# zouyuoz/SVS-UNet-PyTorch

Hardware: AMD Instinct MI355X
Metric: spectrogram-tiles/sec (512x128) U-Net fwd+bwd (L1 train step incl. Adam) (higher is better)
Workload: dtype f32; 1 GPU; train.py L1-loss step, 512x128 tiles, batch 64 per GPU; global_batch=64, parallelism=dp1, mode=train

## Files before the change

### svs_unet_pytorch_amd/csrc/gemm_conv.hip

```cpp
#include <stdlib.h>
#include <string.h>

#include <mutex>
#include <type_traits>
#include <vector>
#include "conv_geom.h"
#include "gemm_pipeline.h"
#include "mfma_split.h"

enum { MODE_GATHER = SVS_MODE_GATHER, MODE_PARITY = SVS_MODE_PARITY };

struct ConvGemmArgs {
  const float* x; long ldx;
  int B, H, W, C;
  const float* wp;
  const float* bias;
  const float* scale;
  const float* shift;
  float slope;
  float* y; long ldy;
  int Ho, Wo, N;
  int accumulate;
  int ksplit;
  float* slab;
// ... 4 lines not shown

struct ConvBal {
  int enabled;
  int npos[4];
  unsigned first[4][65];
  unsigned char nsplit[4][64];
  unsigned char* rowsplit;
};
struct ConvNoBal {};

__device__ __forceinline__ void conv_put(const ConvGemmArgs& p, float v, float* dst, const float* bias, const float* scale, const float* shift,
                                         int n, float& ssum, float& ssq) {
  if (p.bias) v += bias[n];
  if (p.scale) {
    v = v * scale[n] + shift[n];
    v = v > 0.f ? v : v * p.slope;
  }
  if (p.accumulate) v += *dst;
  *dst = v;
  ssum += v;
  ssq += v * v;
}

template <int MODE, int BM, int BN, int WM, int WN, bool UNI, bool SKIP, bool SPLIT, int PF>
__global__ __launch_bounds__(256) void conv_gemm_kernel(ConvGemmArgs p, std::conditional_t<SKIP, ConvBal, ConvNoBal> bal) {
  static_assert(SKIP || !UNI, "the position-uniform form is a form of the tap-skipping kernel");
  constexpr int TM = BM / WM / 16;
  constexpr int TN = BN / WN / 16;
  constexpr int RA = (BM + 63) / 64;
  constexpr int RB = (BN + 63) / 64;
  static_assert(WM * WN == 4, "4 waves");
  static_assert(TM >= 1 && TN >= 1, "tile");

  __shared__ __attribute__((aligned(16))) float As[2][BM * 16];
  __shared__ __attribute__((aligned(16))) float Bs[2][BN * 16];

  const int t = threadIdx.x;
  const int lane = t & 63, wave = t >> 6;
  const int wm = wave / WN, wn = wave % WN;
  const int lrow = lane & 15, q = lane >> 4;

  int bx = blockIdx.x, by = blockIdx.y, bz = blockIdx.z;
  int nsplit = p.ksplit;
  bool balanced = false;
  int upos = -1, ub0 = 0;
  if constexpr (SKIP) {
    if (bal.enabled) {
      balanced = true;
      const unsigned bid = blockIdx.x;
      int c = 0;
      if (MODE == MODE_PARITY) c = (bid >= bal.first[1][0]) + (bid >= bal.first[2][0]) + (bid >= bal.first[3][0]);
      const unsigned f = lane < bal.npos[c] ? bal.first[c][lane] : 0xFFFFFFFFu;
      const int pos = __builtin_amdgcn_readfirstlane(__builtin_popcountll(__ballot(f <= bid)) - 1);
      nsplit = bal.nsplit[c][pos];
      const int ntn = p.N / BN, per = nsplit * ntn;
      const int within = (int)(bid - bal.first[c][pos]);
      const int i = within / per, rem = within - i * per;
      by = rem / ntn;
      bx = (pos * (p.B / BM) + i) * ntn + (rem - by * ntn);
      bz = c;
      upos = pos; ub0 = i * BM;
    }
  }
  const SvsConvClass cls = svs_conv_class<MODE>(bz, p.Ho, p.Wo);
  const int ph = cls.ph, pw = cls.pw, nth = cls.nth, ntw = cls.ntw;
  const int Ha = cls.Ha, Wa = cls.Wa;
  const float* const wp = p.wp + (long)cls.tap0 * p.N * p.C;
  const int ntaps = nth * ntw;
  const long M = (long)p.B * Ha * Wa;
  const int ntile_n = p.N / BN;
  const long m0 = (long)(bx / ntile_n) * BM;
  const int n0 = (bx % ntile_n) * BN;
  if (m0 >= M) {
    if (p.stats && p.ksplit == 1) {
      float* out = p.stats + ((long)bz * (gridDim.x / ntile_n) + bx / ntile_n) * 2 * p.N + n0;
      for (int c = threadIdx.x; c < BN; c += 256) { out[c] = 0.f; out[p.N + c] = 0.f; }
    }
    return;
  }
  const int cpt = p.C >> 4;
  const int nkt = ntaps * cpt;
  int kt_begin = (int)((long)nkt * by / nsplit);
  int kt_end = (int)((long)nkt * (by + 1) / nsplit);
  const long Kw = (long)ntaps * p.C;

  const int chunk = t & 3;
  constexpr unsigned OOB = 0x80000000u;
  unsigned a_voff[RA], a_mask[RA];
  unsigned umask = 0x1FFFFFFu;
  int uhq = 0, uwq = 0;
  if constexpr (UNI) {
    if (upos < 0) {
      upos = (int)((unsigned)m0 / (unsigned)p.B);
      ub0 = (int)((unsigned)m0 - (unsigned)upos * (unsigned)p.B);
    }
    uwq = (int)((unsigned)upos / (unsigned)Ha);
    uhq = upos - uwq * Ha;
    const int h0 = svs_conv_anchor<MODE>(uhq), w0 = svs_conv_anchor<MODE>(uwq);
    umask = svs_tap_mask<MODE>(h0, w0, nth, ntw, p.H, p.W);
    const unsigned base = (unsigned)((((long)h0 * p.W + w0) * p.ldx + chunk * 4) * 4);
    const unsigned per_image = (unsigned)(((long)p.H * p.W * p.ldx) * 4);
#pragma unroll
    for (int r = 0; r < RA; ++r) {
      const int row = (t >> 2) + 64 * r;
      a_voff[r] = (BM % 64 == 0 || row < BM) ? base + (unsigned)(ub0 + row) * per_image : OOB;
      a_mask[r] = 0;
    }
  } else {
#pragma unroll
  for (int r = 0; r < RA; ++r) {
    const int row = (t >> 2) + 64 * r;
    const long m = m0 + row;
    const bool ok = (row < BM) && (m < M);
    const SvsConvRow g = svs_conv_row<SKIP>(ok ? (unsigned)m : 0u, p.B, Ha, Wa);
    const int h0 = svs_conv_anchor<MODE>(g.hq), w0 = svs_conv_anchor<MODE>(g.wq);
    a_voff[r] = ok ? (unsigned)(((((long)g.b * p.H + h0) * p.W + w0) * p.ldx + chunk * 4) * 4) : OOB;
    a_mask[r] = ok ? svs_tap_mask<MODE>(h0, w0, nth, ntw, p.H, p.W) : 0u;
  }
  }
  if (SKIP) {
    if constexpr (!UNI) {
      __shared__ unsigned umask_s;
      if (t == 0) umask_s = 0;
      __syncthreads();
      unsigned mine = 0;
#pragma unroll
      for (int r = 0; r < RA; ++r) mine |= a_mask[r];
      if (mine) atomicOr(&umask_s, mine);
      __syncthreads();
      umask = __builtin_amdgcn_readfirstlane(umask_s);
    }
    if (balanced) {
      const int nvk = __builtin_popcount(umask) << p.cpt_shift;
      const int vb = (int)((long)nvk * by / nsplit), ve = (int)((long)nvk * (by + 1) / nsplit);
      auto kt_of = [&](int v) -> int {
        unsigned m = umask;
        for (int r = v >> p.cpt_shift; r > 0; --r) m &= m - 1;
        return (__builtin_ctz(m) << p.cpt_shift) | (v & (cpt - 1));
      };
      kt_begin = vb < nvk ? kt_of(vb) : nkt;
      kt_end = ve < nvk ? kt_of(ve) : nkt;
    }
  }
  unsigned b_voff[RB];
#pragma unroll
  for (int r = 0; r < RB; ++r) {
    const int row = (t >> 2) + 64 * r;
    b_voff[r] = (row < BN) ? (unsigned)(((long)(n0 + row) * Kw + chunk * 4) * 4) : OOB;
  }
  const __amdgpu_buffer_rsrc_t rx = __builtin_amdgcn_make_buffer_rsrc((void*)(p.x - svs_tap_base_shift<MODE>(p.W, p.ldx)), 0, OOB, 0x00020000);
  const __amdgpu_buffer_rsrc_t rw = __builtin_amdgcn_make_buffer_rsrc((void*)wp, 0, OOB, 0x00020000);

  f32x4 ra[PF][RA], rb[PF][RB];
  auto load_tile = [&](int kt, auto setc) __attribute__((always_inline)) {
    constexpr int set_ = decltype(setc)::value;
    int tap, cc;
    if (SKIP || !p.tap_inner) {
      if (p.cpt_shift >= 0) { tap = kt >> p.cpt_shift; cc = kt & (cpt - 1); }
      else { tap = kt / cpt; cc = kt - tap * cpt; }
    } else {
      cc = (ntaps == 25) ? kt / 25 : (ntaps == 9) ? kt / 9 : (ntaps == 6) ? kt / 6 : kt >> 2;
      tap = kt - cc * ntaps;
    }
    const int th = svs_tap_row(tap, ntw);
    const int tw = tap - th * ntw;
    const int pix = svs_tap_pix<MODE>(th, tw, p.W);
    const int soff_a = __builtin_amdgcn_readfirstlane((int)((pix * p.ldx + (cc << 4)) * 4));
    const int soff_b = __builtin_amdgcn_readfirstlane((int)(((long)tap * p.C + (cc << 4)) * 4));
#pragma unroll
    for (int r = 0; r < RA; ++r) {
      const unsigned vo = (UNI || ((a_mask[r] >> tap) & 1u)) ? a_voff[r] : OOB;
      ra[set_][r] = __builtin_bit_cast(f32x4, __builtin_amdgcn_raw_buffer_load_b128(rx, (int)vo, soff_a, 0));
    }
#pragma unroll
    for (int r = 0; r < RB; ++r)
      rb[set_][r] = __builtin_bit_cast(f32x4, __builtin_amdgcn_raw_buffer_load_b128(rw, (int)b_voff[r], soff_b, 0));
  };
  auto store_tile = [&](int buf, auto setc) __attribute__((always_inline)) {
#pragma unroll
    for (int r = 0; r < RA; ++r) {
      const int row = (t >> 2) + 64 * r;
      if (BM % 64 == 0 || row < BM) *(f32x4*)(&As[buf][row * 16 + swz(row, chunk) * 4]) = ra[decltype(setc)::value][r];
    }
#pragma unroll
    for (int r = 0; r < RB; ++r) {
      const int row = (t >> 2) + 64 * r;
      if (BN % 64 == 0 || row < BN) *(f32x4*)(&Bs[buf][row * 16 + swz(row, chunk) * 4]) = rb[decltype(setc)::value][r];
    }
  };
  f32x4 acc[TM][TN];
#pragma unroll
  for (int i = 0; i < TM; ++i)
#pragma unroll
    for (int j = 0; j < TN; ++j) acc[i][j] = (f32x4){0.f, 0.f, 0.f, 0.f};

  auto first_valid = [&](int k) -> int {
    if (!SKIP || k >= kt_end) return k;
    const int tp = k >> p.cpt_shift;
    if ((umask >> tp) & 1u) return k;
    const unsigned rest = umask >> (tp + 1);
    if (!rest) return kt_end;
    const int nk = (tp + 1 + __builtin_ctz(rest)) << p.cpt_shift;
    return nk < kt_end ? nk : kt_end;
  };
  auto multiply = [&](int buf) __attribute__((always_inline)) {
    f32x4 fa[TM], fb[TN];
#pragma unroll
    for (int i = 0; i < TM; ++i) {
      const int row = wm * (TM * 16) + i * 16 + lrow;
      fa[i] = *(const f32x4*)(&As[buf][row * 16 + swz(row, q) * 4]);
    }
#pragma unroll
    for (int j = 0; j < TN; ++j) {
      const int row = wn * (TN * 16) + j * 16 + lrow;
      fb[j] = *(const f32x4*)(&Bs[buf][row * 16 + swz(row, q) * 4]);
    }
    if constexpr (SPLIT) {
      SvsSplitA sa[TM];
      SvsSplitB sb[TN];
#pragma unroll
      for (int i = 0; i < TM; ++i) sa[i] = svs_split_a(fa[i][0], fa[i][1], fa[i][2], fa[i][3]);
#pragma unroll
      for (int j = 0; j < TN; ++j) sb[j] = svs_split_b(fb[j][0], fb[j][1], fb[j][2], fb[j][3]);
      svs_mma_split<TM, TN>(acc, sa, sb);
    } else {
#pragma unroll
      for (int k = 0; k < 4; ++k)
#pragma unroll
        for (int i = 0; i < TM; ++i)
#pragma unroll
          for (int j = 0; j < TN; ++j)
            acc[i][j] = __builtin_amdgcn_mfma_f32_16x16x4f32(fa[i][k], fb[j][k], acc[i][j], 0, 0, 0);
    }
  };
  svs_k_loop<PF>(first_valid(kt_begin), kt_end, [&](int k) { return first_valid(k + 1); }, load_tile, store_tile, multiply);

  const bool split = p.ksplit > 1;
  float ssum[TN], ssq[TN];
#pragma unroll
  for (int j = 0; j < TN; ++j) { ssum[j] = 0.f; ssq[j] = 0.f; }
  float* const slab = split ? p.slab + (long)by * ((long)p.B * p.Ho * p.Wo) * p.N : nullptr;
  bool mark_rows = false;
  if constexpr (SKIP) mark_rows = balanced && by == 0 && n0 == 0 && wn == 0;
  if constexpr (UNI) {
    const long HoWo = (long)p.Ho * p.Wo;
    const long pix0 = svs_out_pixel<MODE>(0, uhq, uwq, ph, pw, p.Ho, p.Wo) + (long)(ub0 + wm * (TM * 16) + q * 4) * HoWo;
    const int ncol = n0 + wn * (TN * 16) + lrow;
    const long rstride = HoWo * (split ? (long)p.N : p.ldy);
    float* const out = split ? slab + pix0 * p.N + ncol : p.y + pix0 * p.ldy + ncol;
    float cb[TN], csc[TN], csh[TN];
#pragma unroll
    for (int j = 0; j < TN; ++j) {
      cb[j] = (!split && p.bias) ? p.bias[ncol + j * 16] : 0.f;
      csc[j] = (!split && p.scale) ? p.scale[ncol + j * 16] : 0.f;
      csh[j] = (!split && p.scale) ? p.shift[ncol + j * 16] : 0.f;
    }
#pragma unroll
    for (int i = 0; i < TM; ++i) {
#pragma unroll
      for (int r = 0; r < 4; ++r) {
        if (mark_rows && lrow == 0) bal.rowsplit[pix0 + (i * 16 + r) * HoWo] = (unsigned char)nsplit;
        float* const row = out + (i * 16 + r) * rstride;
#pragma unroll
        for (int j = 0; j < TN; ++j) {
          if (split) row[j * 16] = acc[i][j][r];
          else conv_put(p, acc[i][j][r], row + j * 16, cb, csc, csh, j, ssum[j], ssq[j]);
        }
      }
    }
  } else {
#pragma unroll
  for (int i = 0; i < TM; ++i) {
#pragma unroll
    for (int r = 0; r < 4; ++r) {
      const long m = m0 + wm * (TM * 16) + i * 16 + q * 4 + r;
      if (m >= M) continue;
      long opix = m;
      if (SKIP || MODE == MODE_PARITY) {
        const SvsConvRow g = svs_conv_row<SKIP>((unsigned)m, p.B, Ha, Wa);
        opix = svs_out_pixel<MODE>(g.b, g.hq, g.wq, ph, pw, p.Ho, p.Wo);
      }
      if constexpr (SKIP) { if (mark_rows && lrow == 0) bal.rowsplit[opix] = (unsigned char)nsplit; }
#pragma unroll
      for (int j = 0; j < TN; ++j) {
        const int n = n0 + wn * (TN * 16) + j * 16 + lrow;
        if (split) slab[opix * p.N + n] = acc[i][j][r];
        else conv_put(p, acc[i][j][r], p.y + opix * p.ldy + n, p.bias, p.scale, p.shift, n, ssum[j], ssq[j]);
      }
    }
  }
  }
  if (p.stats && !split) {
    __shared__ float st[2][WM][BN];
#pragma unroll
    for (int j = 0; j < TN; ++j) {
      ssum[j] += __shfl_xor(ssum[j], 16, 64); ssum[j] += __shfl_xor(ssum[j], 32, 64);
      ssq[j] += __shfl_xor(ssq[j], 16, 64); ssq[j] += __shfl_xor(ssq[j], 32, 64);
      if (q == 0) { st[0][wm][wn * (TN * 16) + j * 16 + lrow] = ssum[j]; st[1][wm][wn * (TN * 16) + j * 16 + lrow] = ssq[j]; }
    }
    __syncthreads();
    float* out = p.stats + ((long)bz * (gridDim.x / ntile_n) + bx / ntile_n) * 2 * p.N + n0;
    for (int c = t; c < BN; c += 256) {
      float a = 0.f, b2 = 0.f;
#pragma unroll
      for (int w = 0; w < WM; ++w) { a += st[0][w][c]; b2 += st[1][w][c]; }
      out[c] = a;
      out[p.N + c] = b2;
    }
  }
}

template <int MODE, int TM, int TN>
__global__ __launch_bounds__(256) void conv_direct_kernel(ConvGemmArgs p) {
  const int t = threadIdx.x;
  const int lane = t & 63, wave = t >> 6;
  const int lrow = lane & 15, q = lane >> 4;
  const SvsConvClass cls = svs_conv_class<MODE>(blockIdx.y, p.Ho, p.Wo);
  const int ph = cls.ph, pw = cls.pw, nth = cls.nth, ntw = cls.ntw, Ha = cls.Ha, Wa = cls.Wa;
  const float* const wp = p.wp + (long)cls.tap0 * p.N * p.C;
  const int ntaps = nth * ntw;
  const long M = (long)p.B * Ha * Wa;
  const long m0 = ((long)blockIdx.x * 4 + wave) * (TM * 16);
  if (m0 >= M) return;
  const int cpt = p.C >> 4;
  const int nkt = ntaps * cpt;
  const long Kw = (long)ntaps * p.C;
  constexpr unsigned OOB = 0x80000000u;

  unsigned a_voff[TM], a_mask[TM];
#pragma unroll
  for (int i = 0; i < TM; ++i) {
    const long m = m0 + i * 16 + lrow;
    const bool ok = m < M;
    const SvsConvRow g = svs_conv_row<false>(ok ? (unsigned)m : 0u, p.B, Ha, Wa);
    const int h0 = svs_conv_anchor<MODE>(g.hq), w0 = svs_conv_anchor<MODE>(g.wq);
    a_voff[i] = ok ? (unsigned)(((((long)g.b * p.H + h0) * p.W + w0) * p.ldx + q * 4) * 4) : OOB;
    a_mask[i] = ok ? svs_tap_mask<MODE>(h0, w0, nth, ntw, p.H, p.W) : 0u;
  }
  unsigned b_voff[TN];
#pragma unroll
  for (int j = 0; j < TN; ++j) b_voff[j] = (unsigned)(((long)(j * 16 + lrow) * Kw + q * 4) * 4);
  const __amdgpu_buffer_rsrc_t rx = __builtin_amdgcn_make_buffer_rsrc((void*)(p.x - svs_tap_base_shift<MODE>(p.W, p.ldx)), 0, OOB, 0x00020000);
  const __amdgpu_buffer_rsrc_t rw = __builtin_amdgcn_make_buffer_rsrc((void*)wp, 0, OOB, 0x00020000);

  int l_th = 0, l_tw = 0, l_cc = 0;
  auto load_frags = [&](f32x4 (&fa)[TM], f32x4 (&fb)[TN]) {
    const int th = l_th, tw = l_tw, tap = th * ntw + tw;
    const int pix = svs_tap_pix<MODE>(th, tw, p.W);
    const int soff_a = (int)((pix * p.ldx + (l_cc << 4)) * 4);
    const int soff_b = (int)(((long)tap * p.C + (l_cc << 4)) * 4);
    if (++l_tw == ntw) { l_tw = 0; if (++l_th == nth) { l_th = 0; ++l_cc; } }
#pragma unroll
    for (int i = 0; i < TM; ++i) {
      const unsigned vo = ((a_mask[i] >> tap) & 1u) ? a_voff[i] : OOB;
      fa[i] = __builtin_bit_cast(f32x4, __builtin_amdgcn_raw_buffer_load_b128(rx, (int)vo, soff_a, 0));
    }
#pragma unroll
    for (int j = 0; j < TN; ++j)
      fb[j] = __builtin_bit_cast(f32x4, __builtin_amdgcn_raw_buffer_load_b128(rw, (int)b_voff[j], soff_b, 0));
  };
  f32x4 acc[TM][TN];
#pragma unroll
  for (int i = 0; i < TM; ++i)
#pragma unroll
    for (int j = 0; j < TN; ++j) acc[i][j] = (f32x4){0.f, 0.f, 0.f, 0.f};
  auto mma = [&](const f32x4 (&fa)[TM], const f32x4 (&fb)[TN]) {
#pragma unroll
    for (int k = 0; k < 4; ++k)
#pragma unroll
      for (int i = 0; i < TM; ++i)
#pragma unroll
        for (int j = 0; j < TN; ++j)
          acc[i][j] = __builtin_amdgcn_mfma_f32_16x16x4f32(fa[i][k], fb[j][k], acc[i][j], 0, 0, 0);
  };
  f32x4 fa0[TM], fb0[TN], fa1[TM], fb1[TN];
  load_frags(fa0, fb0);
  for (int kt = 0; kt < nkt; kt += 2) {
    if (kt + 1 < nkt) load_frags(fa1, fb1);
    mma(fa0, fb0);
    if (kt + 1 < nkt) {
      if (kt + 2 < nkt) load_frags(fa0, fb0);
      mma(fa1, fb1);
    }
  }
#pragma unroll
  for (int i = 0; i < TM; ++i) {
#pragma unroll
    for (int r = 0; r < 4; ++r) {
// ... 791 lines not shown
```

### svs_unet_pytorch_amd/csrc/gemm_pipeline.h

```cpp
#pragma once
#include <type_traits>

#include "common.h"

template <int PF, class Next, class Fetch, class Store, class Mul>
__device__ __forceinline__ void svs_k_loop(int k, int k_end, Next&& next, Fetch&& fetch, Store&& store, Mul&& multiply) {
  static_assert(PF == 1 || PF == 2, "one or two positions ahead");
  constexpr std::integral_constant<int, 0> set0{};
  constexpr std::integral_constant<int, 1> set1{};
  if constexpr (PF == 2) {
    int k1 = next(k);
    if (k < k_end) fetch(k, set0);
    if (k1 < k_end) fetch(k1, set1);
    if (k < k_end) store(0, set0);
    __syncthreads();
    while (k < k_end) {
      int k2 = next(k1);
      if (k2 < k_end) fetch(k2, set0);
      multiply(0);
      if (k1 < k_end) store(1, set1);
      __syncthreads();
      k = k1; k1 = k2;
      if (k >= k_end) break;
      k2 = next(k1);
      if (k2 < k_end) fetch(k2, set1);
      multiply(1);
      if (k1 < k_end) store(0, set0);
      __syncthreads();
      k = k1; k1 = k2;
    }
  } else {
    if (k < k_end) {
      fetch(k, set0);
      store(0, set0);
    }
    __syncthreads();
    for (int it = 0; k < k_end; ++it) {
      const int buf = it & 1;
      const int kn = next(k);
      const bool more = kn < k_end;
      if (more) fetch(kn, set0);
      k = kn;
      multiply(buf);
      if (more) store(buf ^ 1, set0);
      __syncthreads();
    }
  }
}
```

### svs_unet_pytorch_amd/csrc/gemm_wgrad.hip

```cpp
#include <stdlib.h>

#include "gemm_pipeline.h"
#include "internal.h"
#include "mfma_split.h"

struct WgradArgs {
  const float* s; long lds; int Hs, Ws, Cs;
  const float* l; long ldl; int Hl, Wl, Cl;
  int B;
  float* slab;
  long pix_per_split;
  int ws_shift, hs_shift;
  int b_shift;
};

template <int T> __device__ __forceinline__ void load_vec(const float* p, float (&f)[T]);
template <> __device__ __forceinline__ void load_vec<4>(const float* p, float (&f)[4]) {
  const f32x4 v = *(const f32x4*)p; f[0] = v[0]; f[1] = v[1]; f[2] = v[2]; f[3] = v[3];
}
template <> __device__ __forceinline__ void load_vec<2>(const float* p, float (&f)[2]) {
  const float2 v = *(const float2*)p; f[0] = v.x; f[1] = v.y;
}
template <int T> __device__ __forceinline__ void store_vec(float* p, const float (&f)[T]);
template <> __device__ __forceinline__ void store_vec<4>(float* p, const float (&f)[4]) { *(f32x4*)p = (f32x4){f[0], f[1], f[2], f[3]}; }
template <> __device__ __forceinline__ void store_vec<2>(float* p, const float (&f)[2]) { *(float2*)p = make_float2(f[0], f[1]); }

template <int BM, int BN, int WM, int WN, bool SKIP, bool SPLIT, int PF>
__global__ __launch_bounds__(256) void wgrad_gemm_kernel(WgradArgs p) {
  constexpr int TM = BM / WM / 16;
  constexpr int TN = BN / WN / 16;
  constexpr int LDA = BM + 4, LDB = BN + 4;
  constexpr int CA = BM / 4, CB = BN / 4;
  constexpr int RA = (16 * CA + 255) / 256, RB = (16 * CB + 255) / 256;
  static_assert(WM * WN == 4, "4 waves");

  __shared__ __attribute__((aligned(16))) float As[2][16 * LDA];
  __shared__ __attribute__((aligned(16))) float Bs[2][16 * LDB];

  const int t = threadIdx.x;
  const int lane = t & 63, wave = t >> 6;
  const int wm = wave / WN, wn = wave % WN;
  const int lrow = lane & 15, q = lane >> 4;

  const int Ntot = 25 * p.Cl;
  const int cs0 = blockIdx.x * BM;
  const int n0 = blockIdx.y * BN;
  const long P = (long)p.B * p.Hs * p.Ws;
  const long p_begin = (long)blockIdx.z * p.pix_per_split;
  long p_end = p_begin + p.pix_per_split;
  if (p_end > P) p_end = P;

  constexpr unsigned OOB = 0x80000000u;
  int ak[RA], ac[RA]; bool aok[RA];
#pragma unroll
  for (int r = 0; r < RA; ++r) {
    const int idx = t + 256 * r;
    ak[r] = idx / CA; ac[r] = idx % CA; aok[r] = idx < 16 * CA;
  }
  int bk[RB], bc[RB], bkh[RB], bkw[RB], bcl[RB]; bool bok[RB];
#pragma unroll
  for (int r = 0; r < RB; ++r) {
    const int idx = t + 256 * r;
    bk[r] = idx / CB; bc[r] = idx % CB;
    const int n = n0 + bc[r] * 4;
    bok[r] = (idx < 16 * CB) && (n < Ntot);
    const int tap = bok[r] ? n / p.Cl : 0;
    bcl[r] = bok[r] ? n - tap * p.Cl : 0;
    bkh[r] = tap / 5; bkw[r] = tap - bkh[r] * 5;
  }

  int bj[RB], bi[RB]; unsigned bimg[RB];
#pragma unroll
  for (int r = 0; r < RB; ++r) {
    const unsigned pix = (unsigned)(p_begin + bk[r]);
    const unsigned row = pix / (unsigned)p.Ws;
    bj[r] = (int)(pix - row * (unsigned)p.Ws);
    const unsigned img = row / (unsigned)p.Hs;
    bi[r] = (int)(row - img * (unsigned)p.Hs);
    bimg[r] = img * (unsigned)(p.Hl * p.Wl);
  }
  const unsigned img_stride = (unsigned)(p.Hl * p.Wl);
  auto advance = [&]() {
#pragma unroll
    for (int r = 0; r < RB; ++r) {
      unsigned j = (unsigned)bj[r] + 16u, i = (unsigned)bi[r];
      if (p.ws_shift >= 0) { i += j >> p.ws_shift; j &= (unsigned)p.Ws - 1u; }
      else { const unsigned q = j / (unsigned)p.Ws; j -= q * (unsigned)p.Ws; i += q; }
      unsigned nb;
      if (p.hs_shift >= 0) { nb = i >> p.hs_shift; i &= (unsigned)p.Hs - 1u; }
      else { nb = i / (unsigned)p.Hs; i -= nb * (unsigned)p.Hs; }
      bj[r] = (int)j; bi[r] = (int)i; bimg[r] += nb * img_stride;
    }
  };

  unsigned a_voff[RA];
#pragma unroll
  for (int r = 0; r < RA; ++r) a_voff[r] = aok[r] ? (unsigned)(((long)ak[r] * p.lds + cs0 + ac[r] * 4) * 4) : OOB;
  const __amdgpu_buffer_rsrc_t rs = __builtin_amdgcn_make_buffer_rsrc((void*)(p.s + p_begin * p.lds), 0, OOB, 0x00020000);
  const __amdgpu_buffer_rsrc_t rl = __builtin_amdgcn_make_buffer_rsrc((void*)p.l, 0, OOB, 0x00020000);
  const int HsWs = p.Hs * p.Ws, HlWl = p.Hl * p.Wl;
  unsigned a_voff_s[RA], b_voff_s[RB];
  int tap_lo = 0, tap_hi = 0;
  if (SKIP) {
#pragma unroll
    for (int r = 0; r < RA; ++r) a_voff_s[r] = aok[r] ? (unsigned)((((long)ak[r] * HsWs) * p.lds + cs0 + ac[r] * 4) * 4) : OOB;
#pragma unroll
    for (int r = 0; r < RB; ++r)
      b_voff_s[r] = (unsigned)((((long)bk[r] * HlWl + bkh[r] * p.Wl + bkw[r]) * p.ldl + bcl[r]) * 4);
    tap_lo = n0 / p.Cl;
    const int nlast = (n0 + BN - 1 < Ntot - 1) ? n0 + BN - 1 : Ntot - 1;
    tap_hi = nlast / p.Cl;
  }
  const __amdgpu_buffer_rsrc_t rs_all = __builtin_amdgcn_make_buffer_rsrc((void*)p.s, 0, OOB, 0x00020000);
  const __amdgpu_buffer_rsrc_t rl_sh = __builtin_amdgcn_make_buffer_rsrc((void*)(p.l - (2L * p.Wl + 2) * p.ldl), 0, OOB, 0x00020000);
  auto position = [&](int pk, int& i, int& j, int& b0) {
    const int pos = pk >> p.b_shift;
    b0 = pk & (p.B - 1);
    i = pos >> p.ws_shift;
    j = pos & (p.Ws - 1);
  };
  auto first_valid = [&](int pk) -> int {
    if (!SKIP) return pk;
    while (pk < (int)p_end) {
      int i, j, b0;
      position(pk, i, j, b0);
      bool any = false;
      for (int tp = tap_lo; tp <= tap_hi; ++tp) {
        const int kh = tp / 5, kw = tp - kh * 5;
        any = any || ((unsigned)(2 * i - 2 + kh) < (unsigned)p.Hl && (unsigned)(2 * j - 2 + kw) < (unsigned)p.Wl);
      }
      if (any) return pk;
      pk = ((pk >> p.b_shift) + 1) << p.b_shift;
    }
    return (int)p_end;
  };
  f32x4 ra[PF][RA], rb[PF][RB];
  auto load_tile_skip = [&](int pk, f32x4 (&ra)[RA], f32x4 (&rb)[RB]) __attribute__((always_inline)) {
    int i, j, b0;
    position(pk, i, j, b0);
    const int soff_a = __builtin_amdgcn_readfirstlane((int)((((long)b0 * HsWs + (i * p.Ws + j)) * p.lds) * 4));
    const int soff_b = __builtin_amdgcn_readfirstlane((int)((((long)b0 * HlWl + 2 * i * p.Wl + 2 * j) * p.ldl) * 4));
    const int left = (int)p_end - pk;
#pragma unroll
    for (int r = 0; r < RA; ++r) {
      const unsigned vo = ak[r] < left ? a_voff_s[r] : OOB;
      ra[r] = __builtin_bit_cast(f32x4, __builtin_amdgcn_raw_buffer_load_b128(rs_all, (int)vo, soff_a, 0));
    }
#pragma unroll
    for (int r = 0; r < RB; ++r) {
      const int ih = 2 * i - 2 + bkh[r], iw = 2 * j - 2 + bkw[r];
      const bool ok = bok[r] && bk[r] < left && (unsigned)ih < (unsigned)p.Hl && (unsigned)iw < (unsigned)p.Wl;
      rb[r] = __builtin_bit_cast(f32x4, __builtin_amdgcn_raw_buffer_load_b128(rl_sh, (int)(ok ? b_voff_s[r] : OOB), soff_b, 0));
    }
  };
  auto load_tile = [&](long pk, f32x4 (&ra)[RA], f32x4 (&rb)[RB]) __attribute__((always_inline)) {
    const int soff_a = (int)((pk - p_begin) * p.lds * 4);
    const int left = (int)(p_end - pk);
#pragma unroll
    for (int r = 0; r < RA; ++r) {
      const unsigned vo = ak[r] < left ? a_voff[r] : OOB;
      ra[r] = __builtin_bit_cast(f32x4, __builtin_amdgcn_raw_buffer_load_b128(rs, (int)vo, soff_a, 0));
    }
#pragma unroll
    for (int r = 0; r < RB; ++r) {
      const int ih = 2 * bi[r] - 2 + bkh[r], iw = 2 * bj[r] - 2 + bkw[r];
      const bool ok = bok[r] && bk[r] < left && (unsigned)ih < (unsigned)p.Hl && (unsigned)iw < (unsigned)p.Wl;
      const unsigned vo = ((bimg[r] + (unsigned)(ih * p.Wl + iw)) * (unsigned)p.ldl + (unsigned)bcl[r]) * 4u;
      rb[r] = __builtin_bit_cast(f32x4, __builtin_amdgcn_raw_buffer_load_b128(rl, (int)(ok ? vo : OOB), 0, 0));
    }
    advance();
  };
  auto store_tile = [&](int buf, auto setc) __attribute__((always_inline)) {
    constexpr int set_ = decltype(setc)::value;
#pragma unroll
    for (int r = 0; r < RA; ++r)
      if (aok[r]) *(f32x4*)(&As[buf][ak[r] * LDA + ac[r] * 4]) = ra[set_][r];
#pragma unroll
    for (int r = 0; r < RB; ++r)
      if (t + 256 * r < 16 * CB) *(f32x4*)(&Bs[buf][bk[r] * LDB + bc[r] * 4]) = rb[set_][r];
  };

  f32x4 acc[TM][TN];
#pragma unroll
  for (int i = 0; i < TM; ++i)
#pragma unroll
    for (int j = 0; j < TN; ++j) acc[i][j] = (f32x4){0.f, 0.f, 0.f, 0.f};

  auto multiply = [&](int buf) __attribute__((always_inline)) {
    if constexpr (SPLIT) {
      float ga[4][TM], gb[4][TN];
#pragma unroll
      for (int k = 0; k < 4; ++k) {
        const int kr = 4 * q + k;
        load_vec<TM>(&As[buf][kr * LDA + wm * (TM * 16) + TM * lrow], ga[k]);
        load_vec<TN>(&Bs[buf][kr * LDB + wn * (TN * 16) + TN * lrow], gb[k]);
      }
      SvsSplitA sa[TM];
      SvsSplitB sb[TN];
#pragma unroll
      for (int i = 0; i < TM; ++i) sa[i] = svs_split_a(ga[0][i], ga[1][i], ga[2][i], ga[3][i]);
#pragma unroll
      for (int j = 0; j < TN; ++j) sb[j] = svs_split_b(gb[0][j], gb[1][j], gb[2][j], gb[3][j]);
      svs_mma_split<TM, TN>(acc, sa, sb);
    } else {
#pragma unroll
    for (int k = 0; k < 4; ++k) {
      float fa[TM], fb[TN];
      const int kr = 4 * q + k;
      load_vec<TM>(&As[buf][kr * LDA + wm * (TM * 16) + TM * lrow], fa);
      load_vec<TN>(&Bs[buf][kr * LDB + wn * (TN * 16) + TN * lrow], fb);
#pragma unroll
      for (int i = 0; i < TM; ++i)
#pragma unroll
        for (int j = 0; j < TN; ++j)
          acc[i][j] = __builtin_amdgcn_mfma_f32_16x16x4f32(fa[i], fb[j], acc[i][j], 0, 0, 0);
    }
    }
  };
  auto fetch = [&](int pk, auto setc) __attribute__((always_inline)) {
    constexpr int set_ = decltype(setc)::value;
    if (SKIP) load_tile_skip(pk, ra[set_], rb[set_]);
    else load_tile(pk, ra[set_], rb[set_]);
  };
  svs_k_loop<PF>(first_valid((int)p_begin), (int)p_end, [&](int pk) { return first_valid(pk + 16); }, fetch, store_tile, multiply);

  float* slab = p.slab + (long)blockIdx.z * p.Cs * Ntot;
#pragma unroll
  for (int i = 0; i < TM; ++i)
#pragma unroll
    for (int r = 0; r < 4; ++r) {
      const int cs = cs0 + wm * (TM * 16) + TM * (4 * q + r) + i;
      const int n = n0 + wn * (TN * 16) + TN * lrow;
      if (n < Ntot) {
        float v[TN];
#pragma unroll
        for (int j = 0; j < TN; ++j) v[j] = acc[i][j][r];
        store_vec<TN>(&slab[(long)cs * Ntot + n], v);
      }
    }
}

struct WgWinArgs {
  const float* s; long lds; const float* l; long ldl;
  int B, Hs, Ws, Cs, Hl, Wl, Cl;
  float* slab;
  int ntiles, tiles_per_block;
};

template <int MT>
__global__ __launch_bounds__(256, 2) void wgrad_window_kernel(WgWinArgs p) {
  constexpr int TH = 4, TW = 16, KS = 4 / MT, CSB = 16 * MT;
  constexpr int LS = CSB + 16;
  constexpr int LH = 2 * TH + 3, LW = 2 * TW + 3, LL = 24;
  constexpr int NS = TH * TW * (CSB / 4), NL = LH * LW * 4;
  constexpr int RS = (NS + 255) / 256, RL = (NL + 255) / 256;
  constexpr int KSTEPS = TH * TW / 4 / KS;
  constexpr unsigned OOB = 0x80000000u;
  __shared__ __attribute__((aligned(16))) float Ssm[TH * TW * LS];
  __shared__ __attribute__((aligned(16))) float Lsm[LH * LW * LL];
  const int t = threadIdx.x, lane = t & 63, wave = t >> 6;
  const int lrow = lane & 15, q = lane >> 4;
  const int mt = wave % MT, half = wave / MT;
  const int mchunks = p.Cs / CSB;
  const int m0 = (blockIdx.y % mchunks) * CSB, cl0 = (blockIdx.y / mchunks) * 16;
  const int tiles_w = (p.Ws + TW - 1) / TW, tiles_h = (p.Hs + TH - 1) / TH;
  const int tile_lo = blockIdx.x * p.tiles_per_block;
  const int tile_hi = min(tile_lo + p.tiles_per_block, p.ntiles);

  f32x4 sreg[RS], lreg[RL];
  auto fetch = [&](int tile) {
    const int tw0 = (tile % tiles_w) * TW, th0 = ((tile / tiles_w) % tiles_h) * TH;
    const long b = tile / (tiles_w * tiles_h);
    const __amdgpu_buffer_rsrc_t rs = __builtin_amdgcn_make_buffer_rsrc((void*)(p.s + b * p.Hs * p.Ws * p.lds), 0, OOB, 0x00020000);
    const __amdgpu_buffer_rsrc_t rl = __builtin_amdgcn_make_buffer_rsrc((void*)(p.l + b * p.Hl * p.Wl * p.ldl), 0, OOB, 0x00020000);
#pragma unroll
    for (int r = 0; r < RS; ++r) {
      const int e = t + 256 * r;
      const int c4 = e % (CSB / 4), px = e / (CSB / 4);
      const int sh = th0 + px / TW, sw = tw0 + px % TW;
      const bool ok = e < NS && sh < p.Hs && sw < p.Ws;
      const unsigned vo = ok ? (unsigned)(((sh * p.Ws + sw) * (int)p.lds + m0 + c4 * 4) * 4) : OOB;
      sreg[r] = __builtin_bit_cast(f32x4, __builtin_amdgcn_raw_buffer_load_b128(rs, (int)vo, 0, 0));
    }
#pragma unroll
    for (int r = 0; r < RL; ++r) {
      const int e = t + 256 * r;
      const int c4 = e & 3, px = e >> 2;
      const int ih = 2 * th0 - 2 + px / LW, iw = 2 * tw0 - 2 + px % LW;
      const bool ok = e < NL && (unsigned)ih < (unsigned)p.Hl && (unsigned)iw < (unsigned)p.Wl;
      const unsigned vo = ok ? (unsigned)(((ih * p.Wl + iw) * (int)p.ldl + cl0 + c4 * 4) * 4) : OOB;
      lreg[r] = __builtin_bit_cast(f32x4, __builtin_amdgcn_raw_buffer_load_b128(rl, (int)vo, 0, 0));
    }
  };
  auto stage = [&]() {
#pragma unroll
    for (int r = 0; r < RS; ++r) {
      const int e = t + 256 * r;
      if (e < NS) *(f32x4*)(&Ssm[(e / (CSB / 4)) * LS + (e % (CSB / 4)) * 4]) = sreg[r];
    }
#pragma unroll
    for (int r = 0; r < RL; ++r) {
      const int e = t + 256 * r;
      if (e < NL) *(f32x4*)(&Lsm[(e >> 2) * LL + (e & 3) * 4]) = lreg[r];
    }
  };

  f32x4 acc[25];
#pragma unroll
  for (int i = 0; i < 25; ++i) acc[i] = (f32x4){0.f, 0.f, 0.f, 0.f};
  const float* abase = &Ssm[(half * (TH / KS) * TW + q) * LS + mt * 16 + lrow];
  const float* bbase = &Lsm[(half * (TH / KS) * 2 * LW + 2 * q) * LL + lrow];

  if (tile_lo < tile_hi) fetch(tile_lo);
  for (int tile = tile_lo; tile < tile_hi; ++tile) {
    __syncthreads();
    stage();
    __syncthreads();
    if (tile + 1 < tile_hi) fetch(tile + 1);
#pragma unroll
    for (int ks = 0; ks < KSTEPS; ++ks) {
      const int sh = ks / 4, sg = ks % 4;
      const float a = abase[(sh * TW + sg * 4) * LS];
#pragma unroll
      for (int tap = 0; tap < 25; ++tap) {
        const int kh = tap / 5, kw = tap % 5;
        const float bv = bbase[((2 * sh + kh) * LW + 8 * sg + kw) * LL];
        acc[tap] = __builtin_amdgcn_mfma_f32_16x16x4f32(a, bv, acc[tap], 0, 0, 0);
      }
    }
  }
  const int Ntot = 25 * p.Cl;
  float* slab = p.slab + ((long)blockIdx.x * KS + half) * p.Cs * Ntot;
#pragma unroll
  for (int tap = 0; tap < 25; ++tap)
#pragma unroll
    for (int r = 0; r < 4; ++r)
      slab[(long)(m0 + mt * 16 + 4 * q + r) * Ntot + tap * p.Cl + cl0 + lrow] = acc[tap][r];
}

__global__ __launch_bounds__(256) void wgrad_reduce_kernel(const float* __restrict__ slab, int ksplit, int Cs, int Cl,
                                                           float* __restrict__ dw) {
  __shared__ float tile[25][65];
  const int clt = Cl < 64 ? Cl : 64;
  const int cs = blockIdx.x, cl0 = blockIdx.y * clt;
  const long zstride = (long)Cs * Cl * 25;
  const float* src0 = slab + (long)cs * 25 * Cl + cl0;
  const int q4 = clt >> 2;
  for (int e = threadIdx.x; e < 25 * q4; e += 256) {
    const int tap = e / q4, cl = (e - tap * q4) * 4;
    const float* src = src0 + (long)tap * Cl + cl;
    f32x4 acc = {0.f, 0.f, 0.f, 0.f};
    int z = 0;
    for (; z + 4 <= ksplit; z += 4, src += 4 * zstride) {
      const f32x4 a = *(const f32x4*)src, b = *(const f32x4*)(src + zstride), c = *(const f32x4*)(src + 2 * zstride), d = *(const f32x4*)(src + 3 * zstride);
      acc += a; acc += b; acc += c; acc += d;
    }
    for (; z < ksplit; ++z, src += zstride) acc += *(const f32x4*)src;
    tile[tap][cl] = acc[0]; tile[tap][cl + 1] = acc[1]; tile[tap][cl + 2] = acc[2]; tile[tap][cl + 3] = acc[3];
  }
  __syncthreads();
  float* dst = dw + ((long)cs * Cl + cl0) * 25;
  for (int e = threadIdx.x; e < 25 * clt; e += 256) {
    const int cl = e / 25, tap = e - cl * 25;
    dst[e] = tile[tap][cl];
  }
}

struct WgradTile { int cfg, BM, BN, ksplit; long pps; };
static WgradTile plan_wgrad(int B, int Hs, int Ws, int Cs, int Cl) {
  WgradTile pl{};
  if (Cs % 128 == 0) { pl.cfg = 0; pl.BM = 128; }
  else if (Cs % 64 == 0) { pl.cfg = 1; pl.BM = 64; }
  else { pl.cfg = 2; pl.BM = 32; }
  if (pl.cfg == 0 && ((long)B * Hs * Ws <= 1024 || Cl <= 32)) { pl.cfg = 1; pl.BM = 64; }
  if (svs_tune_on(SVS_TUNE_WGRAD_CFG)) {
    const int c = (int)svs_tune(SVS_TUNE_WGRAD_CFG);
    if (c == 0 && Cs % 128 == 0) { pl.cfg = 0; pl.BM = 128; }
// ... 152 lines not shown
```

Baseline: 20180 tiles/s.

## Add steady-state run loop to GEMM K pipeline skipping per-step validity checks

Adds a fast path to the shared K-loop for fully tiled, non-split PF=2 kernels. Within a run of consecutive valid K positions it issues fetch, multiply and store with no bounds or next() checks. The conv kernel gets a cheaper tap/channel decode (umulhi reciprocal division and a multiply-shift for the tap row), and the wgrad kernel gets a run_end helper built on a factored any_tap test. Guards that are compile-time true are also folded away. The goal is less scalar and branch overhead per K step, at the cost of more code size and subtle invariants in the run-boundary logic.

```diff
diff --git a/svs_unet_pytorch_amd/csrc/gemm_conv.hip b/svs_unet_pytorch_amd/csrc/gemm_conv.hip
--- a/svs_unet_pytorch_amd/csrc/gemm_conv.hip
+++ b/svs_unet_pytorch_amd/csrc/gemm_conv.hip
@@ -180,8 +180,22 @@
   const __amdgpu_buffer_rsrc_t rw = __builtin_amdgcn_make_buffer_rsrc((void*)wp, 0, OOB, 0x00020000);
 
   f32x4 ra[PF][RA], rb[PF][RB];
+  auto load_taps = [&](int tap, int th, int cc, auto setc) __attribute__((always_inline)) {
+    constexpr int set_ = decltype(setc)::value;
+    const int tw = tap - th * ntw;
+    const int pix = svs_tap_pix<MODE>(th, tw, p.W);
+    const int soff_a = __builtin_amdgcn_readfirstlane((int)((pix * p.ldx + (cc << 4)) * 4));
+    const int soff_b = __builtin_amdgcn_readfirstlane((int)(((long)tap * p.C + (cc << 4)) * 4));
+#pragma unroll
+    for (int r = 0; r < RA; ++r) {
+      const unsigned vo = (UNI || ((a_mask[r] >> tap) & 1u)) ? a_voff[r] : OOB;
+      ra[set_][r] = __builtin_bit_cast(f32x4, __builtin_amdgcn_raw_buffer_load_b128(rx, (int)vo, soff_a, 0));
+    }
+#pragma unroll
+    for (int r = 0; r < RB; ++r)
+      rb[set_][r] = __builtin_bit_cast(f32x4, __builtin_amdgcn_raw_buffer_load_b128(rw, (int)b_voff[r], soff_b, 0));
+  };
   auto load_tile = [&](int kt, auto setc) __attribute__((always_inline)) {
-    constexpr int set_ = decltype(setc)::value;
     int tap, cc;
     if (SKIP || !p.tap_inner) {
       if (p.cpt_shift >= 0) { tap = kt >> p.cpt_shift; cc = kt & (cpt - 1); }
@@ -190,19 +204,21 @@
       cc = (ntaps == 25) ? kt / 25 : (ntaps == 9) ? kt / 9 : (ntaps == 6) ? kt / 6 : kt >> 2;
       tap = kt - cc * ntaps;
     }
-    const int th = svs_tap_row(tap, ntw);
-    const int tw = tap - th * ntw;
-    const int pix = svs_tap_pix<MODE>(th, tw, p.W);
-    const int soff_a = __builtin_amdgcn_readfirstlane((int)((pix * p.ldx + (cc << 4)) * 4));
-    const int soff_b = __builtin_amdgcn_readfirstlane((int)(((long)tap * p.C + (cc << 4)) * 4));
-#pragma unroll
-    for (int r = 0; r < RA; ++r) {
-      const unsigned vo = (UNI || ((a_mask[r] >> tap) & 1u)) ? a_voff[r] : OOB;
-      ra[set_][r] = __builtin_bit_cast(f32x4, __builtin_amdgcn_raw_buffer_load_b128(rx, (int)vo, soff_a, 0));
-    }
-#pragma unroll
-    for (int r = 0; r < RB; ++r)
-      rb[set_][r] = __builtin_bit_cast(f32x4, __builtin_amdgcn_raw_buffer_load_b128(rw, (int)b_voff[r], soff_b, 0));
+    load_taps(tap, svs_tap_row(tap, ntw), cc, setc);
+  };
+  const bool tap_outer = SKIP || !p.tap_inner;
+  const unsigned kdiv = tap_outer ? (unsigned)cpt : (unsigned)ntaps;
+  const bool runs_ok = SKIP || (unsigned long)nkt * kdiv < (1ul << 32);
+  const unsigned kmul = SKIP ? 0u : 0xFFFFFFFFu / kdiv + 1u;
+  const int kone = kdiv == 1u ? -1 : 0, kouter = tap_outer ? -1 : 0;
+  const int rowmul = ntw == 5 ? 52 : ntw == 3 ? 86 : 128;
+  auto load_tile_run = [&](int kt, auto setc) __attribute__((always_inline)) {
+    int a;
+    if constexpr (SKIP) a = kt >> p.cpt_shift;
+    else a = (int)__umulhi((unsigned)kt, kmul) + (kt & kone);
+    const int b = kt - a * (int)kdiv;
+    const int tap = SKIP ? a : (a & kouter) | (b & ~kouter), cc = SKIP ? b : (b & kouter) | (a & ~kouter);
+    load_taps(tap, (tap * rowmul) >> 8, cc, setc);
   };
   auto store_tile = [&](int buf, auto setc) __attribute__((always_inline)) {
 #pragma unroll
@@ -261,7 +277,14 @@
             acc[i][j] = __builtin_amdgcn_mfma_f32_16x16x4f32(fa[i][k], fb[j][k], acc[i][j], 0, 0, 0);
     }
   };
-  svs_k_loop<PF>(first_valid(kt_begin), kt_end, [&](int k) { return first_valid(k + 1); }, load_tile, store_tile, multiply);
+  auto run_end = [&](int k) -> int {
+    if (!SKIP) return runs_ok ? kt_end : k + 1;
+    const int tp = k >> p.cpt_shift;
+    const int e = (tp + __builtin_ctz(~(umask >> tp))) << p.cpt_shift;
+    return e < kt_end ? e : kt_end;
+  };
+  svs_k_loop<PF, BM, BN, SPLIT>(first_valid(kt_begin), kt_end, 1, [&](int k) { return first_valid(k + 1); }, run_end, load_tile, load_tile_run, store_tile,
+                 multiply);
 
   const bool split = p.ksplit > 1;
   float ssum[TN], ssq[TN];
diff --git a/svs_unet_pytorch_amd/csrc/gemm_pipeline.h b/svs_unet_pytorch_amd/csrc/gemm_pipeline.h
--- a/svs_unet_pytorch_amd/csrc/gemm_pipeline.h
+++ b/svs_unet_pytorch_amd/csrc/gemm_pipeline.h
@@ -3,12 +3,55 @@
 
 #include "common.h"
 
-template <int PF, class Next, class Fetch, class Store, class Mul>
-__device__ __forceinline__ void svs_k_loop(int k, int k_end, Next&& next, Fetch&& fetch, Store&& store, Mul&& multiply) {
+constexpr bool svs_k_loop_steady(int BM, int BN, bool split) { return BM % 64 == 0 && BN % 64 == 0 && !split; }
+
+template <int PF, int BM, int BN, bool SPLIT, class Next, class RunEnd, class Fetch, class FetchRun, class Store, class Mul>
+__device__ __forceinline__ void svs_k_loop(int k, int k_end, int step, Next&& next, RunEnd&& run_end, Fetch&& fetch, FetchRun&& fetch_run,
+                                           Store&& store, Mul&& multiply) {
   static_assert(PF == 1 || PF == 2, "one or two positions ahead");
   constexpr std::integral_constant<int, 0> set0{};
   constexpr std::integral_constant<int, 1> set1{};
-  if constexpr (PF == 2) {
+  if constexpr (PF == 2 && svs_k_loop_steady(BM, BN, SPLIT)) {
+    if (k < k_end) {
+      int k1 = next(k);
+      fetch(k, set0);
+      if (k1 < k_end) fetch(k1, set1);
+      store(0, set0);
+      __syncthreads();
+      int re = run_end(k);
+      do {
+        if (k >= re) re = run_end(k);
+        if (k + 3 * step < re) {
+          do {
+            fetch_run(k + 2 * step, set0);
+            multiply(0);
+            store(1, set1);
+            __syncthreads();
+            fetch_run(k + 3 * step, set1);
+            multiply(1);
+            store(0, set0);
+            __syncthreads();
+            k += 2 * step;
+          } while (k + 3 * step < re);
+          k1 = k + step;
+        }
+        int k2 = next(k1);
+        if (k2 < k_end) fetch(k2, set0);
+        multiply(0);
+        if (k1 < k_end) store(1, set1);
+        __syncthreads();
+        k = k1; k1 = k2;
+        if (k < k_end) {
+          k2 = next(k1);
+          if (k2 < k_end) fetch(k2, set1);
+          multiply(1);
+          store(0, set0);
+          __syncthreads();
+          k = k1; k1 = k2;
+        }
+      } while (k < k_end);
+    }
+  } else if constexpr (PF == 2) {
     int k1 = next(k);
     if (k < k_end) fetch(k, set0);
     if (k1 < k_end) fetch(k1, set1);
diff --git a/svs_unet_pytorch_amd/csrc/gemm_wgrad.hip b/svs_unet_pytorch_amd/csrc/gemm_wgrad.hip
--- a/svs_unet_pytorch_amd/csrc/gemm_wgrad.hip
+++ b/svs_unet_pytorch_amd/csrc/gemm_wgrad.hip
@@ -55,7 +55,7 @@
 #pragma unroll
   for (int r = 0; r < RA; ++r) {
     const int idx = t + 256 * r;
-    ak[r] = idx / CA; ac[r] = idx % CA; aok[r] = idx < 16 * CA;
+    ak[r] = idx / CA; ac[r] = idx % CA; aok[r] = (16 * CA) % 256 == 0 || idx < 16 * CA;
   }
   int bk[RB], bc[RB], bkh[RB], bkw[RB], bcl[RB]; bool bok[RB];
 #pragma unroll
@@ -119,20 +119,29 @@
     i = pos >> p.ws_shift;
     j = pos & (p.Ws - 1);
   };
+  auto any_tap = [&](int pk) -> bool {
+    int i, j, b0;
+    position(pk, i, j, b0);
+    bool any = false;
+    for (int tp = tap_lo; tp <= tap_hi; ++tp) {
+      const int kh = tp / 5, kw = tp - kh * 5;
+      any = any || ((unsigned)(2 * i - 2 + kh) < (unsigned)p.Hl && (unsigned)(2 * j - 2 + kw) < (unsigned)p.Wl);
+    }
+    return any;
+  };
   auto first_valid = [&](int pk) -> int {
     if (!SKIP) return pk;
     while (pk < (int)p_end) {
-      int i, j, b0;
-      position(pk, i, j, b0);
-      bool any = false;
-      for (int tp = tap_lo; tp <= tap_hi; ++tp) {
-        const int kh = tp / 5, kw = tp - kh * 5;
-        any = any || ((unsigned)(2 * i - 2 + kh) < (unsigned)p.Hl && (unsigned)(2 * j - 2 + kw) < (unsigned)p.Wl);
-      }
-      if (any) return pk;
+      if (any_tap(pk)) return pk;
       pk = ((pk >> p.b_shift) + 1) << p.b_shift;
     }
     return (int)p_end;
+  };
+  auto run_end = [&](int pk) -> int {
+    if (!SKIP) return (int)p_end;
+    do pk = ((pk >> p.b_shift) + 1) << p.b_shift;
+    while (pk < (int)p_end && any_tap(pk));
+    return __builtin_amdgcn_readfirstlane(pk < (int)p_end ? pk : (int)p_end);
   };
   f32x4 ra[PF][RA], rb[PF][RB];
   auto load_tile_skip = [&](int pk, f32x4 (&ra)[RA], f32x4 (&rb)[RB]) __attribute__((always_inline)) {
@@ -149,7 +158,7 @@
 #pragma unroll
     for (int r = 0; r < RB; ++r) {
       const int ih = 2 * i - 2 + bkh[r], iw = 2 * j - 2 + bkw[r];
-      const bool ok = bok[r] && bk[r] < left && (unsigned)ih < (unsigned)p.Hl && (unsigned)iw < (unsigned)p.Wl;
+      const bool ok = bok[r] & (bk[r] < left) & ((unsigned)ih < (unsigned)p.Hl) & ((unsigned)iw < (unsigned)p.Wl);
       rb[r] = __builtin_bit_cast(f32x4, __builtin_amdgcn_raw_buffer_load_b128(rl_sh, (int)(ok ? b_voff_s[r] : OOB), soff_b, 0));
     }
   };
@@ -177,7 +186,7 @@
       if (aok[r]) *(f32x4*)(&As[buf][ak[r] * LDA + ac[r] * 4]) = ra[set_][r];
 #pragma unroll
     for (int r = 0; r < RB; ++r)
-      if (t + 256 * r < 16 * CB) *(f32x4*)(&Bs[buf][bk[r] * LDB + bc[r] * 4]) = rb[set_][r];
+      if ((16 * CB) % 256 == 0 || t + 256 * r < 16 * CB) *(f32x4*)(&Bs[buf][bk[r] * LDB + bc[r] * 4]) = rb[set_][r];
   };
 
   f32x4 acc[TM][TN];
@@ -222,7 +231,8 @@
     if (SKIP) load_tile_skip(pk, ra[set_], rb[set_]);
     else load_tile(pk, ra[set_], rb[set_]);
   };
-  svs_k_loop<PF>(first_valid((int)p_begin), (int)p_end, [&](int pk) { return first_valid(pk + 16); }, fetch, store_tile, multiply);
+  svs_k_loop<PF, BM, BN, SPLIT>(__builtin_amdgcn_readfirstlane(first_valid((int)p_begin)), (int)p_end, 16, [&](int pk) { return first_valid(pk + 16); }, run_end, fetch, fetch, store_tile,
+                 multiply);
 
   float* slab = p.slab + (long)blockIdx.z * p.Cs * Ntot;
 #pragma unroll
```

Result: no change. 20210 tiles/s, median of 2 (+0.1%).
